# OFA-Sys/ONE-PEACE

Measured on NVIDIA H100. Metric: encoder_samples_per_sec, higher is better.
Workload: dtype bf16

## Files before the change

one_peace_b200/csrc/attention_wgmma.cu:

```cuda
#include "common.cuh"
#include "gemm.h"
#include "ops.h"

namespace opb {
namespace {

constexpr int kHd = 64;
constexpr int kThreads = 384;
constexpr int kStagerThreads = 96;
constexpr int kBoxRows = 32;
constexpr int kBoxBytes = kBoxRows * 128;
constexpr int kKeyChunks = kAttnShortMaxS / 32;

constexpr int kOffQ = 0;
constexpr int kOffK = kOffQ + 4 * 64 * 128;
constexpr int kOffV = kOffK + kAttnShortMaxS * 128;
constexpr int kOffLut = kOffV + kAttnShortMaxS * 128;
constexpr int kOffPad = kOffLut + kAttnShortMaxLut * 4;
constexpr int kBufBytes = (kOffPad + kAttnShortMaxS + 1023) / 1024 * 1024;
constexpr int kOffCodes = 2 * kBufBytes;
constexpr int kOffBars = kOffCodes + 2 * kAttnShortMaxS * 4;
constexpr int kSmemBytes = kOffBars + 64 + 1024;
static_assert(kSmemBytes <= 227 * 1024, "one CTA per SM");

enum BiasForm : int { kNoBias = 0, kDense = 1, kLut = 2, kLutSeg = 3 };

struct ShortArgs {
  const float* bias;
  long bias_bstride;
  int s_pad;
  LutBias lb;
  const uint8_t* key_pad;
  __nv_bfloat16* out;
  float* lse;
  float* ln_stats;
  int B, S, H;
};

OPB_DEVICE void wgmma_m64n32k16_ss(float (&d)[16], uint64_t desc_a, uint64_t desc_b, uint32_t scale_d) {
  asm volatile(
      "{\n\t"
      ".reg .pred p;\n\t"
      "setp.ne.b32 p, %18, 0;\n\t"
      "wgmma.mma_async.sync.aligned.m64n32k16.f32.bf16.bf16 "
      "{%0, %1, %2, %3, %4, %5, %6, %7, %8, %9, %10, %11, %12, %13, %14, %15}, %16, %17, p, 1, 1, 0, 0;\n\t"
      "}\n"
      : "+f"(d[0]), "+f"(d[1]), "+f"(d[2]), "+f"(d[3]), "+f"(d[4]), "+f"(d[5]), "+f"(d[6]), "+f"(d[7]),
        "+f"(d[8]), "+f"(d[9]), "+f"(d[10]), "+f"(d[11]), "+f"(d[12]), "+f"(d[13]), "+f"(d[14]), "+f"(d[15])
      : "l"(desc_a), "l"(desc_b), "r"(scale_d));
}

OPB_DEVICE void wgmma_m64n64k16_rs(float (&d)[32], const uint32_t (&a)[4], uint64_t desc_b, uint32_t scale_d) {
  asm volatile(
      "{\n\t"
      ".reg .pred p;\n\t"
      "setp.ne.b32 p, %37, 0;\n\t"
      "wgmma.mma_async.sync.aligned.m64n64k16.f32.bf16.bf16 "
      "{%0, %1, %2, %3, %4, %5, %6, %7, %8, %9, %10, %11, %12, %13, %14, %15, "
      "%16, %17, %18, %19, %20, %21, %22, %23, %24, %25, %26, %27, %28, %29, %30, %31}, "
      "{%32, %33, %34, %35}, %36, p, 1, 1, 1;\n\t"
      "}\n"
      : "+f"(d[0]), "+f"(d[1]), "+f"(d[2]), "+f"(d[3]), "+f"(d[4]), "+f"(d[5]), "+f"(d[6]), "+f"(d[7]),
        "+f"(d[8]), "+f"(d[9]), "+f"(d[10]), "+f"(d[11]), "+f"(d[12]), "+f"(d[13]), "+f"(d[14]), "+f"(d[15]),
        "+f"(d[16]), "+f"(d[17]), "+f"(d[18]), "+f"(d[19]), "+f"(d[20]), "+f"(d[21]), "+f"(d[22]), "+f"(d[23]),
        "+f"(d[24]), "+f"(d[25]), "+f"(d[26]), "+f"(d[27]), "+f"(d[28]), "+f"(d[29]), "+f"(d[30]), "+f"(d[31])
      : "r"(a[0]), "r"(a[1]), "r"(a[2]), "r"(a[3]), "l"(desc_b), "r"(scale_d));
}

template <int N>
OPB_DEVICE void fence_regs(float (&d)[N]) {
#pragma unroll
  for (int i = 0; i < N; ++i) asm volatile("" : "+f"(d[i])::"memory");
}

OPB_DEVICE float quad_max(float v) {
  v = fmaxf(v, __shfl_xor_sync(0xffffffffu, v, 1));
  return fmaxf(v, __shfl_xor_sync(0xffffffffu, v, 2));
}
OPB_DEVICE float quad_sum(float v) {
  v += __shfl_xor_sync(0xffffffffu, v, 1);
  return v + __shfl_xor_sync(0xffffffffu, v, 2);
}

OPB_DEVICE void load_bias_chunk(float2 (&dst)[4][2], const float* bias_lo, const float* bias_hi, int c, int t, int S) {
#pragma unroll
  for (int j = 0; j < 4; ++j) {
    const int key = (4 * c + j) * 8 + 2 * t;
    dst[j][0] = key < S ? *reinterpret_cast<const float2*>(bias_lo + key) : make_float2(0.f, 0.f);
    dst[j][1] = key < S ? *reinterpret_cast<const float2*>(bias_hi + key) : make_float2(0.f, 0.f);
  }
}

template <int kForm, int kChunks>
OPB_DEVICE void attend_tile(const ShortArgs& a, const uint8_t* buf, const int* code_row_s, const int* code_col_s, int b,
                            int h, int qt) {
  const int S = a.S, D = a.H * kHd;
  const int warp = (threadIdx.x >> 5) & 3, lane = threadIdx.x & 31;
  const int g = lane >> 2, t = lane & 3;
  const int row_lo = qt * 64 + warp * 16 + g, row_hi = row_lo + 8;
  const int rl = row_lo < S ? row_lo : 0, rh = row_hi < S ? row_hi : 0;
  const bool warp_live = qt * 64 + warp * 16 < S;

  const float* bias_lo = nullptr;
  const float* bias_hi = nullptr;
  float2 pre[2][4][2];
  if (kForm == kDense && warp_live) {
    bias_lo = a.bias + b * a.bias_bstride + (static_cast<long>(h) * S + rl) * a.s_pad;
    bias_hi = a.bias + b * a.bias_bstride + (static_cast<long>(h) * S + rh) * a.s_pad;
    load_bias_chunk(pre[0], bias_lo, bias_hi, 0, t, S);
    if (kChunks > 1) load_bias_chunk(pre[1], bias_lo, bias_hi, 1, t, S);
  }

  float s[kChunks][16];
  const uint32_t q_addr = smem_u32(buf + kOffQ) + qt * 8192;
  const uint32_t k_addr = smem_u32(buf + kOffK);
  wgmma_fence();
#pragma unroll
  for (int c = 0; c < kChunks; ++c) {
#pragma unroll
    for (int k = 0; k < 4; ++k)
      wgmma_m64n32k16_ss(s[c], wgmma_desc_sw128(q_addr + 32 * k, 8192), wgmma_desc_sw128(k_addr + c * 4096 + 32 * k, 8192),
                         k > 0 ? 1u : 0u);
  }
  wgmma_commit();
  wgmma_wait<0>();
#pragma unroll
  for (int c = 0; c < kChunks; ++c) fence_regs(s[c]);

  float mx_lo = -INFINITY, mx_hi = -INFINITY, sum_lo = 0.f, sum_hi = 0.f;
  uint32_t pf[4 * kChunks][2];
  if (warp_live) {
    const uint8_t* kp = a.key_pad != nullptr ? buf + kOffPad : nullptr;
    const float* lut_s = reinterpret_cast<const float*>(buf + kOffLut);
    const int crow_lo = kForm >= kLut ? code_row_s[rl] : 0;
    const int crow_hi = kForm >= kLut ? code_row_s[rh] : 0;
    const int seg = a.lb.seg_split;
    const bool first_lo = rl < seg, first_hi = rh < seg;
#pragma unroll
    for (int nt = 0; nt < 4 * kChunks; ++nt) {
      const int c = nt >> 2, e = (nt & 3) * 4;
      const int key = nt * 8 + 2 * t;
      float b00 = 0.f, b01 = 0.f, b10 = 0.f, b11 = 0.f;
      if (kForm == kDense) {
        if ((nt & 3) == 0) __syncwarp();
        const float2 x = pre[c & 1][nt & 3][0], y = pre[c & 1][nt & 3][1];
        b00 = x.x; b01 = x.y; b10 = y.x; b11 = y.y;
        if ((nt & 3) == 3 && c + 2 < kChunks) load_bias_chunk(pre[c & 1], bias_lo, bias_hi, c + 2, t, S);
      } else if (kForm == kLut) {
        const int2 cc = *reinterpret_cast<const int2*>(code_col_s + key);
        b00 = lut_s[crow_lo - cc.x]; b01 = lut_s[crow_lo - cc.y];
        b10 = lut_s[crow_hi - cc.x]; b11 = lut_s[crow_hi - cc.y];
      } else if (kForm == kLutSeg) {
        const int2 cc = *reinterpret_cast<const int2*>(code_col_s + key);
        const bool kf0 = key < seg, kf1 = key + 1 < seg;
        const bool s00 = first_lo == kf0, s01 = first_lo == kf1, s10 = first_hi == kf0, s11 = first_hi == kf1;
        b00 = lut_s[s00 ? crow_lo - cc.x : 0]; b01 = lut_s[s01 ? crow_lo - cc.y : 0];
        b10 = lut_s[s10 ? crow_hi - cc.x : 0]; b11 = lut_s[s11 ? crow_hi - cc.y : 0];
        b00 = s00 ? b00 : 0.f; b01 = s01 ? b01 : 0.f;
        b10 = s10 ? b10 : 0.f; b11 = s11 ? b11 : 0.f;
      }
      bool dead0 = key >= S, dead1 = key + 1 >= S;
      if (kp != nullptr) {
        const uint32_t pair = *reinterpret_cast<const uint16_t*>(kp + key);
        dead0 = dead0 || (pair & 0xffu) != 0;
        dead1 = dead1 || (pair >> 8) != 0;
      }
      s[c][e + 0] = dead0 ? -INFINITY : s[c][e + 0] + b00;
      s[c][e + 1] = dead1 ? -INFINITY : s[c][e + 1] + b01;
      s[c][e + 2] = dead0 ? -INFINITY : s[c][e + 2] + b10;
      s[c][e + 3] = dead1 ? -INFINITY : s[c][e + 3] + b11;
      mx_lo = fmaxf(mx_lo, fmaxf(s[c][e + 0], s[c][e + 1]));
      mx_hi = fmaxf(mx_hi, fmaxf(s[c][e + 2], s[c][e + 3]));
    }
    mx_lo = quad_max(mx_lo);
    mx_hi = quad_max(mx_hi);

    const float base_lo = (mx_lo == -INFINITY) ? 0.f : mx_lo;
    const float base_hi = (mx_hi == -INFINITY) ? 0.f : mx_hi;
#pragma unroll
    for (int nt = 0; nt < 4 * kChunks; ++nt) {
      const int c = nt >> 2, e = (nt & 3) * 4;
      const float p0 = __expf(s[c][e + 0] - base_lo), p1 = __expf(s[c][e + 1] - base_lo);
      const float p2 = __expf(s[c][e + 2] - base_hi), p3 = __expf(s[c][e + 3] - base_hi);
      sum_lo += p0 + p1;
      sum_hi += p2 + p3;
      pf[nt][0] = pack_bf16x2(p0, p1);
      pf[nt][1] = pack_bf16x2(p2, p3);
    }
  } else {
#pragma unroll
    for (int nt = 0; nt < 4 * kChunks; ++nt) pf[nt][0] = pf[nt][1] = 0u;
  }

  float o[32];
  const uint32_t v_addr = smem_u32(buf + kOffV);
#pragma unroll
  for (int nt = 0; nt < 4 * kChunks; ++nt) asm volatile("" : "+r"(pf[nt][0]), "+r"(pf[nt][1])::"memory");
  fence_regs(o);
  wgmma_fence();
#pragma unroll
  for (int kk = 0; kk < 2 * kChunks; ++kk) {
    const uint32_t af[4] = {pf[2 * kk][0], pf[2 * kk][1], pf[2 * kk + 1][0], pf[2 * kk + 1][1]};
    wgmma_m64n64k16_rs(o, af, wgmma_desc_sw128(v_addr + kk * 2048, 8192), kk > 0 ? 1u : 0u);
  }
  wgmma_commit();
  wgmma_wait<0>();
  fence_regs(o);

  const float l_lo = quad_sum(sum_lo), l_hi = quad_sum(sum_hi);
  const float inv_lo = l_lo > 0.f ? 1.f / l_lo : 0.f;
  const float inv_hi = l_hi > 0.f ? 1.f / l_hi : 0.f;
  const long rows_total = static_cast<long>(a.B) * S;
  if (a.ln_stats != nullptr) {
    float s_lo = 0.f, q_lo = 0.f, s_hi = 0.f, q_hi = 0.f;
#pragma unroll
    for (int nd = 0; nd < 8; ++nd) {
      const float a0 = o[4 * nd] * inv_lo, a1 = o[4 * nd + 1] * inv_lo;
      const float a2 = o[4 * nd + 2] * inv_hi, a3 = o[4 * nd + 3] * inv_hi;
      s_lo += a0 + a1; q_lo += a0 * a0 + a1 * a1;
      s_hi += a2 + a3; q_hi += a2 * a2 + a3 * a3;
    }
    s_lo = quad_sum(s_lo); q_lo = quad_sum(q_lo);
    s_hi = quad_sum(s_hi); q_hi = quad_sum(q_hi);
    if (t == 0 && row_lo < S)
      *reinterpret_cast<float2*>(a.ln_stats + (h * rows_total + static_cast<long>(b) * S + row_lo) * 2) = make_float2(s_lo, q_lo);
    if (t == 0 && row_hi < S)
      *reinterpret_cast<float2*>(a.ln_stats + (h * rows_total + static_cast<long>(b) * S + row_hi) * 2) = make_float2(s_hi, q_hi);
  }
  if (row_lo < S) {
    __nv_bfloat16* op = a.out + (static_cast<long>(b) * S + row_lo) * D + h * kHd + 2 * t;
#pragma unroll
    for (int nd = 0; nd < 8; ++nd)
      *reinterpret_cast<uint32_t*>(op + nd * 8) = pack_bf16x2(o[4 * nd] * inv_lo, o[4 * nd + 1] * inv_lo);
    if (a.lse != nullptr && t == 0) a.lse[(static_cast<long>(b) * a.H + h) * S + row_lo] = mx_lo + __logf(l_lo);
  }
  if (row_hi < S) {
    __nv_bfloat16* op = a.out + (static_cast<long>(b) * S + row_hi) * D + h * kHd + 2 * t;
#pragma unroll
    for (int nd = 0; nd < 8; ++nd)
      *reinterpret_cast<uint32_t*>(op + nd * 8) = pack_bf16x2(o[4 * nd + 2] * inv_hi, o[4 * nd + 3] * inv_hi);
    if (a.lse != nullptr && t == 0) a.lse[(static_cast<long>(b) * a.H + h) * S + row_hi] = mx_hi + __logf(l_hi);
  }
}

template <int kForm, int kChunks>
__global__ void __launch_bounds__(kThreads, 1)
attention_short_kernel(const __grid_constant__ CUtensorMap tm_qkv, const ShortArgs a) {
  extern __shared__ uint8_t smem_raw[];
  uint8_t* smem = smem_raw + ((1024u - (smem_u32(smem_raw) & 1023u)) & 1023u);
  int* code_row_s = reinterpret_cast<int*>(smem + kOffCodes);
  int* code_col_s = code_row_s + kAttnShortMaxS;
  uint64_t* full = reinterpret_cast<uint64_t*>(smem + kOffBars);
  uint64_t* empty = full + 2;

  const int S = a.S, H = a.H, D = H * kHd;
  const int units = a.B * H;
  const int n_qt = (S + 63) / 64;
  const int wg = threadIdx.x >> 7;

  if (threadIdx.x == 0) {
    tma_prefetch_desc(&tm_qkv);
    for (int i = 0; i < 2; ++i) {
      mbar_init(&full[i], 1 + kStagerThreads);
      mbar_init(&empty[i], 8);
    }
    fence_barrier_init();
  }
  if (kForm >= kLut) {
    for (int i = threadIdx.x; i < kAttnShortMaxS; i += kThreads) {
      if (i < S) code_row_s[i] = a.lb.code_row[i];
      code_col_s[i] = a.lb.code_col[i < S ? i : S - 1];
    }
  }
  __syncthreads();

  if (wg == 0) {
    asm volatile("setmaxnreg.dec.sync.aligned.u32 40;");
    if (threadIdx.x == 0) {
      uint32_t j = 0;
      for (int unit = blockIdx.x; unit < units; unit += gridDim.x, ++j) {
        const int b = unit / H, h = unit - b * H;
        uint8_t* buf = smem + (j & 1) * kBufBytes;
        mbar_wait_quiet(&empty[j & 1], ((j >> 1) & 1) ^ 1);
        mbar_arrive_expect_tx(&full[j & 1], 3 * kChunks * kBoxBytes);
        for (int i = 0; i < kChunks; ++i) {
          tma_load_3d(&tm_qkv, &full[j & 1], buf + kOffQ + i * kBoxBytes, h * kHd, i * kBoxRows, b);
          tma_load_3d(&tm_qkv, &full[j & 1], buf + kOffK + i * kBoxBytes, D + h * kHd, i * kBoxRows, b);
          tma_load_3d(&tm_qkv, &full[j & 1], buf + kOffV + i * kBoxBytes, 2 * D + h * kHd, i * kBoxRows, b);
        }
      }
    } else if (threadIdx.x >= 32) {
      const int t = threadIdx.x - 32;
      uint32_t j = 0;
      for (int unit = blockIdx.x; unit < units; unit += gridDim.x, ++j) {
        const int b = unit / H, h = unit - b * H;
        uint8_t* buf = smem + (j & 1) * kBufBytes;
        mbar_wait_quiet(&empty[j & 1], ((j >> 1) & 1) ^ 1);
        if (kForm >= kLut) {
          const float* src = a.lb.lut + static_cast<long>(h) * a.lb.lut_len;
          float* dst = reinterpret_cast<float*>(buf + kOffLut);
          for (int i = t; i < a.lb.lut_len; i += kStagerThreads) dst[i] = src[i];
        }
        if (a.key_pad != nullptr) {
          const uint8_t* src = a.key_pad + static_cast<long>(b) * S;
          for (int i = t; i < S; i += kStagerThreads) buf[kOffPad + i] = src[i];
        }
        mbar_arrive(&full[j & 1]);
      }
    }
  } else {
    asm volatile("setmaxnreg.inc.sync.aligned.u32 232;");
    const int cw = wg - 1;
    uint32_t j = 0;
    for (int unit = blockIdx.x; unit < units; unit += gridDim.x, ++j) {
      const int b = unit / H, h = unit - b * H;
      const uint8_t* buf = smem + (j & 1) * kBufBytes;
      mbar_wait_quiet(&full[j & 1], (j >> 1) & 1);
      for (int qt = cw; qt < n_qt; qt += 2) attend_tile<kForm, kChunks>(a, buf, code_row_s, code_col_s, b, h, qt);
      __syncwarp();
      if ((threadIdx.x & 31) == 0) mbar_arrive(&empty[j & 1]);
    }
  }
}

template <int kForm, int kChunks>
int launch_short(const CUtensorMap& tm, const ShortArgs& a, cudaStream_t stream) {
  auto kern = attention_short_kernel<kForm, kChunks>;
  static bool attr_set = false;
  if (!attr_set) {
    if (cudaFuncSetAttribute(kern, cudaFuncAttributeMaxDynamicSharedMemorySize, kSmemBytes) != cudaSuccess)
      return OPB_ERR_CUDA;
    attr_set = true;
  }
  const int units = a.B * a.H;
  const int grid = units < sm_count() ? units : sm_count();
  kern<<<grid, kThreads, kSmemBytes, stream>>>(tm, a);
  return cudaGetLastError() == cudaSuccess ? OPB_OK : OPB_ERR_CUDA;
}

template <int kForm>
int launch_form(const CUtensorMap& tm, const ShortArgs& a, cudaStream_t stream) {
  static_assert(kKeyChunks == 7, "one case per chunk count");
  switch ((a.S + 31) / 32) {
    case 1: return launch_short<kForm, 1>(tm, a, stream);
    case 2: return launch_short<kForm, 2>(tm, a, stream);
    case 3: return launch_short<kForm, 3>(tm, a, stream);
    case 4: return launch_short<kForm, 4>(tm, a, stream);
    case 5: return launch_short<kForm, 5>(tm, a, stream);
    case 6: return launch_short<kForm, 6>(tm, a, stream);
    case 7: return launch_short<kForm, 7>(tm, a, stream);
    default: return OPB_ERR_INVALID;
  }
}

}

int attention_fwd_short(const void* qkv, const float* bias, const uint8_t* key_pad, void* out, float* lse, float* ln_stats,
                        int B, int S, int H, int s_pad, long bias_bstride, const LutBias& lb, cudaStream_t stream) {
  if (B <= 0 || S <= 0 || H <= 0 || S > kAttnShortMaxS || lb.lut_len > kAttnShortMaxLut) return OPB_ERR_INVALID;
  const uint64_t D = static_cast<uint64_t>(H) * kHd;
  CUtensorMap tm;
  const int rc = make_tmap_bf16_batched(&tm, qkv, 3 * D, S, 3 * D, B, S * 3 * D, kBoxRows);
  if (rc != OPB_OK) return rc;
  ShortArgs a;
  a.bias = bias; a.bias_bstride = bias_bstride; a.s_pad = s_pad; a.lb = lb;
  a.key_pad = key_pad;
  a.out = reinterpret_cast<__nv_bfloat16*>(out); a.lse = lse; a.ln_stats = ln_stats;
  a.B = B; a.S = S; a.H = H;
  if (bias != nullptr) return launch_form<kDense>(tm, a, stream);
  if (lb.lut != nullptr) return lb.seg_split > 0 ? launch_form<kLutSeg>(tm, a, stream) : launch_form<kLut>(tm, a, stream);
  return launch_form<kNoBias>(tm, a, stream);
}

}
```

one_peace_b200/csrc/common.cuh:

```cuda
#pragma once
#include <cuda.h>
#include <cuda_bf16.h>
#include <cuda_runtime.h>
#include <stdint.h>
#include <stdio.h>
#include <stdlib.h>

#define OPB_DEVICE __device__ __forceinline__

#define OPB_OK 0
#define OPB_ERR_INVALID 1
#define OPB_ERR_CUDA 2
#define OPB_ERR_UNSUPPORTED 3

namespace opb {

OPB_DEVICE uint32_t smem_u32(const void* p) {
  return static_cast<uint32_t>(__cvta_generic_to_shared(p));
}
OPB_DEVICE uint32_t lane_id() { return threadIdx.x & 31; }

OPB_DEVICE bool elect_one() {
  uint32_t pred = 0;
  asm volatile(
      "{\n\t"
      ".reg .pred P;\n\t"
      "elect.sync _|P, 0xffffffff;\n\t"
      "selp.b32 %0, 1, 0, P;\n\t"
      "}\n"
      : "=r"(pred));
  return pred != 0;
}

OPB_DEVICE uint64_t globaltimer_ns() {
  uint64_t t;
  asm volatile("mov.u64 %0, %%globaltimer;" : "=l"(t));
  return t;
}

OPB_DEVICE void mbar_init(uint64_t* bar, uint32_t count) {
  asm volatile("mbarrier.init.shared::cta.b64 [%0], %1;" ::"r"(smem_u32(bar)), "r"(count) : "memory");
}
OPB_DEVICE void fence_barrier_init() { asm volatile("fence.mbarrier_init.release.cluster;" ::: "memory"); }
OPB_DEVICE void fence_proxy_async() { asm volatile("fence.proxy.async.shared::cta;" ::: "memory"); }

OPB_DEVICE void mbar_arrive_expect_tx(uint64_t* bar, uint32_t bytes) {
  asm volatile("mbarrier.arrive.expect_tx.shared::cta.b64 _, [%0], %1;" ::"r"(smem_u32(bar)), "r"(bytes)
               : "memory");
}
OPB_DEVICE void mbar_arrive(uint64_t* bar) {
  asm volatile("mbarrier.arrive.shared::cta.b64 _, [%0];" ::"r"(smem_u32(bar)) : "memory");
}
OPB_DEVICE void mbar_arrive_count(uint64_t* bar, uint32_t count) {
  asm volatile("mbarrier.arrive.shared::cta.b64 _, [%0], %1;" ::"r"(smem_u32(bar)), "r"(count) : "memory");
}
OPB_DEVICE bool mbar_try_wait(uint64_t* bar, uint32_t parity) {
  uint32_t ok;
  asm volatile(
      "{\n\t"
      ".reg .pred P;\n\t"
      "mbarrier.try_wait.parity.shared::cta.b64 P, [%1], %2;\n\t"
      "selp.b32 %0, 1, 0, P;\n\t"
      "}\n"
      : "=r"(ok)
      : "r"(smem_u32(bar)), "r"(parity)
      : "memory");
  return ok != 0;
}

#ifndef OPB_WATCHDOG_NS
#define OPB_WATCHDOG_NS 4000000000ull
#endif
OPB_DEVICE void mbar_wait(uint64_t* bar, uint32_t parity) {
  if (mbar_try_wait(bar, parity)) return;
  uint64_t t0 = globaltimer_ns();
  uint32_t spins = 0;
  while (!mbar_try_wait(bar, parity)) {
    if ((++spins & 0x3ff) == 0) {
      if (globaltimer_ns() - t0 > OPB_WATCHDOG_NS) {
        printf("[opb] mbarrier watchdog: block %d thread %d bar@%u parity %u\n", (int)blockIdx.x,
               (int)threadIdx.x, smem_u32(bar), parity);
        __trap();
      }
    }
  }
}

OPB_DEVICE void mbar_wait_quiet(uint64_t* bar, uint32_t parity) {
  if (mbar_try_wait(bar, parity)) return;
  const uint64_t t0 = globaltimer_ns();
  while (!mbar_try_wait(bar, parity)) {
    if (globaltimer_ns() - t0 > OPB_WATCHDOG_NS) __trap();
  }
}

OPB_DEVICE uint64_t wgmma_desc_sw128(uint32_t smem_addr, uint32_t lbo) {
  uint64_t d = 0;
  d |= static_cast<uint64_t>((smem_addr & 0x3FFFFu) >> 4);
  d |= static_cast<uint64_t>((lbo >> 4) & 0x3FFFu) << 16;
  d |= static_cast<uint64_t>(1024 >> 4) << 32;
  d |= static_cast<uint64_t>(1) << 62;
  return d;
}

OPB_DEVICE void wgmma_fence() { asm volatile("wgmma.fence.sync.aligned;" ::: "memory"); }
OPB_DEVICE void wgmma_commit() { asm volatile("wgmma.commit_group.sync.aligned;" ::: "memory"); }
template <int N>
OPB_DEVICE void wgmma_wait() { asm volatile("wgmma.wait_group.sync.aligned %0;" ::"n"(N) : "memory"); }

static inline int sm_count() {
  static int n = 0;
  if (n == 0) {
    int dev = 0;
    cudaGetDevice(&dev);
    cudaDeviceGetAttribute(&n, cudaDevAttrMultiProcessorCount, dev);
  }
  return n;
}

OPB_DEVICE void tma_prefetch_desc(const CUtensorMap* m) {
  asm volatile("prefetch.tensormap [%0];" ::"l"(reinterpret_cast<uint64_t>(m)) : "memory");
}

OPB_DEVICE void tma_load_2d(const CUtensorMap* m, uint64_t* bar, void* dst, int32_t c0, int32_t c1) {
  asm volatile(
      "cp.async.bulk.tensor.2d.shared::cluster.global.mbarrier::complete_tx::bytes [%0], [%1, {%3, %4}], [%2];"
      :
      : "r"(smem_u32(dst)), "l"(reinterpret_cast<uint64_t>(m)), "r"(smem_u32(bar)), "r"(c0), "r"(c1)
      : "memory");
}
OPB_DEVICE void tma_load_3d(const CUtensorMap* m, uint64_t* bar, void* dst, int32_t c0, int32_t c1, int32_t c2) {
  asm volatile(
      "cp.async.bulk.tensor.3d.shared::cluster.global.mbarrier::complete_tx::bytes [%0], [%1, {%3, %4, %5}], [%2];"
      :
      : "r"(smem_u32(dst)), "l"(reinterpret_cast<uint64_t>(m)), "r"(smem_u32(bar)), "r"(c0), "r"(c1), "r"(c2)
      : "memory");
}
OPB_DEVICE void bulk_load_1d(void* dst, const void* src, uint32_t bytes, uint64_t* bar) {
  asm volatile("cp.async.bulk.shared::cluster.global.mbarrier::complete_tx::bytes [%0], [%1], %2, [%3];" ::"r"(smem_u32(dst)),
               "l"(reinterpret_cast<uint64_t>(src)), "r"(bytes), "r"(smem_u32(bar))
               : "memory");
}

OPB_DEVICE void tma_store_2d(const CUtensorMap* m, const void* src, int32_t c0, int32_t c1) {
  asm volatile("cp.async.bulk.tensor.2d.global.shared::cta.bulk_group [%0, {%2, %3}], [%1];" ::"l"(
                   reinterpret_cast<uint64_t>(m)),
               "r"(smem_u32(src)), "r"(c0), "r"(c1)
               : "memory");
}
OPB_DEVICE void bulk_commit() { asm volatile("cp.async.bulk.commit_group;" ::: "memory"); }
template <int N>
OPB_DEVICE void bulk_wait_read() { asm volatile("cp.async.bulk.wait_group.read %0;" ::"n"(N) : "memory"); }
template <int N>
OPB_DEVICE void bulk_wait_all() { asm volatile("cp.async.bulk.wait_group %0;" ::"n"(N) : "memory"); }

OPB_DEVICE uint32_t sw64_off(int row, int chunk) { return row * 64 + ((chunk ^ ((row >> 1) & 3)) << 4); }
OPB_DEVICE uint32_t sw128_off(int row, int chunk) { return row * 128 + ((chunk ^ (row & 7)) << 4); }

OPB_DEVICE float fast_erf(float x) {
  const float ax = fabsf(x);
  float t;
  asm("rcp.approx.ftz.f32 %0, %1;" : "=f"(t) : "f"(fmaf(0.3275911f, ax, 1.0f)));
  float p = fmaf(1.061405429f, t, -1.453152027f);
  p = fmaf(p, t, 1.421413741f);
  p = fmaf(p, t, -0.284496736f);
  p = fmaf(p, t, 0.254829592f);
  p *= t;
  float e;
  asm("ex2.approx.ftz.f32 %0, %1;" : "=f"(e) : "f"(-1.4426950408889634f * ax * ax));
  const float r = fmaf(-p, e, 1.0f);
  return copysignf(r, x);
}
OPB_DEVICE float gelu_erf(float x) { return 0.5f * x * (1.0f + fast_erf(x * 0.70710678118654752440f)); }

OPB_DEVICE float4 lds128(const uint8_t* p) { return *reinterpret_cast<const float4*>(p); }
OPB_DEVICE void sts128(uint8_t* p, float4 v) { *reinterpret_cast<float4*>(p) = v; }
OPB_DEVICE void sts128u(uint8_t* p, uint4 v) { *reinterpret_cast<uint4*>(p) = v; }

OPB_DEVICE uint32_t pack_bf16x2(float lo, float hi) {
  __nv_bfloat162 v = __floats2bfloat162_rn(lo, hi);
  return *reinterpret_cast<uint32_t*>(&v);
}
OPB_DEVICE float2 unpack_bf16x2(uint32_t u) {
  __nv_bfloat162 v = *reinterpret_cast<__nv_bfloat162*>(&u);
  return __bfloat1622float2(v);
}

OPB_DEVICE float warp_sum(float v) {
#pragma unroll
  for (int o = 16; o > 0; o >>= 1) v += __shfl_xor_sync(0xffffffffu, v, o);
  return v;
}
OPB_DEVICE float warp_max(float v) {
#pragma unroll
  for (int o = 16; o > 0; o >>= 1) v = fmaxf(v, __shfl_xor_sync(0xffffffffu, v, o));
  return v;
}

}
```

Before: 830.0.

## Store attention output via stmatrix and TMA, specialize key-pad masking

The attention output epilogue now writes each 64-row tile into the consumed Q buffer in shared memory with stmatrix using a 128B swizzle, then issues one TMA 3D store per warpgroup in place of scattered 4-byte global stores. The bias/mask loop is also split into compile-time variants with and without key padding, and the out-of-range key check is limited to the last chunk. LUT addressing is simplified, and q-tile assignment alternates between consumer warpgroups across units. The change adds a named barrier and a bulk wait before releasing the buffer, and it relies on the TMA box clipping rows past S.

New measurement: 833.9 (median of 6 runs). About the same (+0.5%).

```diff
diff --git a/one_peace_b200/csrc/attention_wgmma.cu b/one_peace_b200/csrc/attention_wgmma.cu
--- a/one_peace_b200/csrc/attention_wgmma.cu
+++ b/one_peace_b200/csrc/attention_wgmma.cu
@@ -1,3 +1,5 @@
+#include <type_traits>
+
 #include "common.cuh"
 #include "gemm.h"
 #include "ops.h"
@@ -92,9 +94,9 @@
 }
 
 template <int kForm, int kChunks>
-OPB_DEVICE void attend_tile(const ShortArgs& a, const uint8_t* buf, const int* code_row_s, const int* code_col_s, int b,
-                            int h, int qt) {
-  const int S = a.S, D = a.H * kHd;
+OPB_DEVICE void attend_tile(const CUtensorMap& tm_out, const ShortArgs& a, const uint8_t* buf, const int* code_row_s,
+                            const int* code_col_s, int b, int h, int qt) {
+  const int S = a.S;
   const int warp = (threadIdx.x >> 5) & 3, lane = threadIdx.x & 31;
   const int g = lane >> 2, t = lane & 3;
   const int row_lo = qt * 64 + warp * 16 + g, row_hi = row_lo + 8;
@@ -136,42 +138,50 @@
     const int crow_hi = kForm >= kLut ? code_row_s[rh] : 0;
     const int seg = a.lb.seg_split;
     const bool first_lo = rl < seg, first_hi = rh < seg;
-#pragma unroll
-    for (int nt = 0; nt < 4 * kChunks; ++nt) {
-      const int c = nt >> 2, e = (nt & 3) * 4;
-      const int key = nt * 8 + 2 * t;
-      float b00 = 0.f, b01 = 0.f, b10 = 0.f, b11 = 0.f;
-      if (kForm == kDense) {
-        if ((nt & 3) == 0) __syncwarp();
-        const float2 x = pre[c & 1][nt & 3][0], y = pre[c & 1][nt & 3][1];
-        b00 = x.x; b01 = x.y; b10 = y.x; b11 = y.y;
-        if ((nt & 3) == 3 && c + 2 < kChunks) load_bias_chunk(pre[c & 1], bias_lo, bias_hi, c + 2, t, S);
-      } else if (kForm == kLut) {
-        const int2 cc = *reinterpret_cast<const int2*>(code_col_s + key);
-        b00 = lut_s[crow_lo - cc.x]; b01 = lut_s[crow_lo - cc.y];
-        b10 = lut_s[crow_hi - cc.x]; b11 = lut_s[crow_hi - cc.y];
-      } else if (kForm == kLutSeg) {
-        const int2 cc = *reinterpret_cast<const int2*>(code_col_s + key);
-        const bool kf0 = key < seg, kf1 = key + 1 < seg;
-        const bool s00 = first_lo == kf0, s01 = first_lo == kf1, s10 = first_hi == kf0, s11 = first_hi == kf1;
-        b00 = lut_s[s00 ? crow_lo - cc.x : 0]; b01 = lut_s[s01 ? crow_lo - cc.y : 0];
-        b10 = lut_s[s10 ? crow_hi - cc.x : 0]; b11 = lut_s[s11 ? crow_hi - cc.y : 0];
-        b00 = s00 ? b00 : 0.f; b01 = s01 ? b01 : 0.f;
-        b10 = s10 ? b10 : 0.f; b11 = s11 ? b11 : 0.f;
+    const float* lut_lo = lut_s + crow_lo;
+    const float* lut_hi = lut_s + crow_hi;
+    auto bias_mask_max = [&](auto has_pad) {
+      const bool pad = has_pad;
+#pragma unroll
+      for (int nt = 0; nt < 4 * kChunks; ++nt) {
+        const int c = nt >> 2, e = (nt & 3) * 4;
+        const int key = nt * 8 + 2 * t;
+        float b00 = 0.f, b01 = 0.f, b10 = 0.f, b11 = 0.f;
+        if (kForm == kDense) {
+          if ((nt & 3) == 0) __syncwarp();
+          const float2 x = pre[c & 1][nt & 3][0], y = pre[c & 1][nt & 3][1];
+          b00 = x.x; b01 = x.y; b10 = y.x; b11 = y.y;
+          if ((nt & 3) == 3 && c + 2 < kChunks) load_bias_chunk(pre[c & 1], bias_lo, bias_hi, c + 2, t, S);
+        } else if (kForm == kLut) {
+          const int2 cc = *reinterpret_cast<const int2*>(code_col_s + key);
+          b00 = lut_lo[-cc.x]; b01 = lut_lo[-cc.y];
+          b10 = lut_hi[-cc.x]; b11 = lut_hi[-cc.y];
+        } else if (kForm == kLutSeg) {
+          const int2 cc = *reinterpret_cast<const int2*>(code_col_s + key);
+          const bool kf0 = key < seg, kf1 = key + 1 < seg;
+          const bool s00 = first_lo == kf0, s01 = first_lo == kf1, s10 = first_hi == kf0, s11 = first_hi == kf1;
+          b00 = *(s00 ? lut_lo - cc.x : lut_s); b01 = *(s01 ? lut_lo - cc.y : lut_s);
+          b10 = *(s10 ? lut_hi - cc.x : lut_s); b11 = *(s11 ? lut_hi - cc.y : lut_s);
+          b00 = s00 ? b00 : 0.f; b01 = s01 ? b01 : 0.f;
+          b10 = s10 ? b10 : 0.f; b11 = s11 ? b11 : 0.f;
+        }
+        bool dead0 = c == kChunks - 1 && key >= S, dead1 = c == kChunks - 1 && key + 1 >= S;
+        if (pad) {
+          const uint32_t pair = *reinterpret_cast<const uint16_t*>(kp + key);
+          dead0 = dead0 || (pair & 0xffu) != 0;
+          dead1 = dead1 || (pair >> 8) != 0;
+        }
+        s[c][e + 0] = dead0 ? -INFINITY : s[c][e + 0] + b00;
+        s[c][e + 1] = dead1 ? -INFINITY : s[c][e + 1] + b01;
+        s[c][e + 2] = dead0 ? -INFINITY : s[c][e + 2] + b10;
+        s[c][e + 3] = dead1 ? -INFINITY : s[c][e + 3] + b11;
+        mx_lo = fmaxf(mx_lo, fmaxf(s[c][e + 0], s[c][e + 1]));
+        mx_hi = fmaxf(mx_hi, fmaxf(s[c][e + 2], s[c][e + 3]));
       }
-      bool dead0 = key >= S, dead1 = key + 1 >= S;
-      if (kp != nullptr) {
-        const uint32_t pair = *reinterpret_cast<const uint16_t*>(kp + key);
-        dead0 = dead0 || (pair & 0xffu) != 0;
-        dead1 = dead1 || (pair >> 8) != 0;
-      }
-      s[c][e + 0] = dead0 ? -INFINITY : s[c][e + 0] + b00;
-      s[c][e + 1] = dead1 ? -INFINITY : s[c][e + 1] + b01;
-      s[c][e + 2] = dead0 ? -INFINITY : s[c][e + 2] + b10;
-      s[c][e + 3] = dead1 ? -INFINITY : s[c][e + 3] + b11;
-      mx_lo = fmaxf(mx_lo, fmaxf(s[c][e + 0], s[c][e + 1]));
-      mx_hi = fmaxf(mx_hi, fmaxf(s[c][e + 2], s[c][e + 3]));
-    }
+    };
+    if constexpr (kForm == kDense) bias_mask_max(kp != nullptr);
+    else if (kp != nullptr) bias_mask_max(std::true_type{});
+    else bias_mask_max(std::false_type{});
     mx_lo = quad_max(mx_lo);
     mx_hi = quad_max(mx_hi);
 
@@ -227,25 +237,39 @@
     if (t == 0 && row_hi < S)
       *reinterpret_cast<float2*>(a.ln_stats + (h * rows_total + static_cast<long>(b) * S + row_hi) * 2) = make_float2(s_hi, q_hi);
   }
-  if (row_lo < S) {
-    __nv_bfloat16* op = a.out + (static_cast<long>(b) * S + row_lo) * D + h * kHd + 2 * t;
-#pragma unroll
-    for (int nd = 0; nd < 8; ++nd)
-      *reinterpret_cast<uint32_t*>(op + nd * 8) = pack_bf16x2(o[4 * nd] * inv_lo, o[4 * nd + 1] * inv_lo);
-    if (a.lse != nullptr && t == 0) a.lse[(static_cast<long>(b) * a.H + h) * S + row_lo] = mx_lo + __logf(l_lo);
-  }
-  if (row_hi < S) {
-    __nv_bfloat16* op = a.out + (static_cast<long>(b) * S + row_hi) * D + h * kHd + 2 * t;
-#pragma unroll
-    for (int nd = 0; nd < 8; ++nd)
-      *reinterpret_cast<uint32_t*>(op + nd * 8) = pack_bf16x2(o[4 * nd + 2] * inv_hi, o[4 * nd + 3] * inv_hi);
-    if (a.lse != nullptr && t == 0) a.lse[(static_cast<long>(b) * a.H + h) * S + row_hi] = mx_hi + __logf(l_hi);
+  if (a.lse != nullptr && t == 0) {
+    if (row_lo < S) a.lse[(static_cast<long>(b) * a.H + h) * S + row_lo] = mx_lo + __logf(l_lo);
+    if (row_hi < S) a.lse[(static_cast<long>(b) * a.H + h) * S + row_hi] = mx_hi + __logf(l_hi);
+  }
+
+  uint8_t* stage = const_cast<uint8_t*>(buf) + kOffQ + qt * 8192;
+#pragma unroll
+  for (int half = 0; half < 2; ++half) {
+    const float inv = half ? inv_hi : inv_lo;
+    const int row = warp * 16 + 8 * half + (lane & 7);
+#pragma unroll
+    for (int q = 0; q < 2; ++q) {
+      uint32_t v[4];
+#pragma unroll
+      for (int i = 0; i < 4; ++i) v[i] = pack_bf16x2(o[4 * (4 * q + i) + 2 * half] * inv, o[4 * (4 * q + i) + 2 * half + 1] * inv);
+      const uint32_t addr = smem_u32(stage) + sw128_off(row, 4 * q + (lane >> 3));
+      asm volatile("stmatrix.sync.aligned.m8n8.x4.shared.b16 [%0], {%1, %2, %3, %4};" ::"r"(addr), "r"(v[0]), "r"(v[1]),
+                   "r"(v[2]), "r"(v[3]));
+    }
+  }
+  fence_proxy_async();
+  if (threadIdx.x >> 7 == 1) asm volatile("bar.sync 1, 128;" ::: "memory");
+  else asm volatile("bar.sync 2, 128;" ::: "memory");
+  if ((threadIdx.x & 127) == 0) {
+    tma_store_3d(&tm_out, stage, h * kHd, qt * 64, b);
+    bulk_commit();
   }
 }
 
 template <int kForm, int kChunks>
 __global__ void __launch_bounds__(kThreads, 1)
-attention_short_kernel(const __grid_constant__ CUtensorMap tm_qkv, const ShortArgs a) {
+attention_short_kernel(const __grid_constant__ CUtensorMap tm_qkv, const __grid_constant__ CUtensorMap tm_out,
+                       const ShortArgs a) {
   extern __shared__ uint8_t smem_raw[];
   uint8_t* smem = smem_raw + ((1024u - (smem_u32(smem_raw) & 1023u)) & 1023u);
   int* code_row_s = reinterpret_cast<int*>(smem + kOffCodes);
@@ -260,6 +284,7 @@
 
   if (threadIdx.x == 0) {
     tma_prefetch_desc(&tm_qkv);
+    tma_prefetch_desc(&tm_out);
     for (int i = 0; i < 2; ++i) {
       mbar_init(&full[i], 1 + kStagerThreads);
       mbar_init(&empty[i], 8);
@@ -316,7 +341,9 @@
       const int b = unit / H, h = unit - b * H;
       const uint8_t* buf = smem + (j & 1) * kBufBytes;
       mbar_wait_quiet(&full[j & 1], (j >> 1) & 1);
-      for (int qt = cw; qt < n_qt; qt += 2) attend_tile<kForm, kChunks>(a, buf, code_row_s, code_col_s, b, h, qt);
+      for (int qt = (cw + j) & 1; qt < n_qt; qt += 2)
+        attend_tile<kForm, kChunks>(tm_out, a, buf, code_row_s, code_col_s, b, h, qt);
+      if ((threadIdx.x & 127) == 0) bulk_wait_read<0>();
       __syncwarp();
       if ((threadIdx.x & 31) == 0) mbar_arrive(&empty[j & 1]);
     }
@@ -324,7 +351,7 @@
 }
 
 template <int kForm, int kChunks>
-int launch_short(const CUtensorMap& tm, const ShortArgs& a, cudaStream_t stream) {
+int launch_short(const CUtensorMap& tm, const CUtensorMap& tm_out, const ShortArgs& a, cudaStream_t stream) {
   auto kern = attention_short_kernel<kForm, kChunks>;
   static bool attr_set = false;
   if (!attr_set) {
@@ -334,21 +361,21 @@
   }
   const int units = a.B * a.H;
   const int grid = units < sm_count() ? units : sm_count();
-  kern<<<grid, kThreads, kSmemBytes, stream>>>(tm, a);
+  kern<<<grid, kThreads, kSmemBytes, stream>>>(tm, tm_out, a);
   return cudaGetLastError() == cudaSuccess ? OPB_OK : OPB_ERR_CUDA;
 }
 
 template <int kForm>
-int launch_form(const CUtensorMap& tm, const ShortArgs& a, cudaStream_t stream) {
+int launch_form(const CUtensorMap& tm, const CUtensorMap& tm_out, const ShortArgs& a, cudaStream_t stream) {
   static_assert(kKeyChunks == 7, "one case per chunk count");
   switch ((a.S + 31) / 32) {
-    case 1: return launch_short<kForm, 1>(tm, a, stream);
-    case 2: return launch_short<kForm, 2>(tm, a, stream);
-    case 3: return launch_short<kForm, 3>(tm, a, stream);
-    case 4: return launch_short<kForm, 4>(tm, a, stream);
-    case 5: return launch_short<kForm, 5>(tm, a, stream);
-    case 6: return launch_short<kForm, 6>(tm, a, stream);
-    case 7: return launch_short<kForm, 7>(tm, a, stream);
+    case 1: return launch_short<kForm, 1>(tm, tm_out, a, stream);
+    case 2: return launch_short<kForm, 2>(tm, tm_out, a, stream);
+    case 3: return launch_short<kForm, 3>(tm, tm_out, a, stream);
+    case 4: return launch_short<kForm, 4>(tm, tm_out, a, stream);
+    case 5: return launch_short<kForm, 5>(tm, tm_out, a, stream);
+    case 6: return launch_short<kForm, 6>(tm, tm_out, a, stream);
+    case 7: return launch_short<kForm, 7>(tm, tm_out, a, stream);
     default: return OPB_ERR_INVALID;
   }
 }
@@ -360,16 +387,20 @@
   if (B <= 0 || S <= 0 || H <= 0 || S > kAttnShortMaxS || lb.lut_len > kAttnShortMaxLut) return OPB_ERR_INVALID;
   const uint64_t D = static_cast<uint64_t>(H) * kHd;
   CUtensorMap tm;
-  const int rc = make_tmap_bf16_batched(&tm, qkv, 3 * D, S, 3 * D, B, S * 3 * D, kBoxRows);
+  int rc = make_tmap_bf16_batched(&tm, qkv, 3 * D, S, 3 * D, B, S * 3 * D, kBoxRows);
+  if (rc != OPB_OK) return rc;
+  CUtensorMap tm_out;
+  rc = make_tmap_bf16_batched(&tm_out, out, D, S, D, B, S * D, 64);
   if (rc != OPB_OK) return rc;
   ShortArgs a;
   a.bias = bias; a.bias_bstride = bias_bstride; a.s_pad = s_pad; a.lb = lb;
   a.key_pad = key_pad;
   a.out = reinterpret_cast<__nv_bfloat16*>(out); a.lse = lse; a.ln_stats = ln_stats;
   a.B = B; a.S = S; a.H = H;
-  if (bias != nullptr) return launch_form<kDense>(tm, a, stream);
-  if (lb.lut != nullptr) return lb.seg_split > 0 ? launch_form<kLutSeg>(tm, a, stream) : launch_form<kLut>(tm, a, stream);
-  return launch_form<kNoBias>(tm, a, stream);
-}
-
-}
+  if (bias != nullptr) return launch_form<kDense>(tm, tm_out, a, stream);
+  if (lb.lut != nullptr)
+    return lb.seg_split > 0 ? launch_form<kLutSeg>(tm, tm_out, a, stream) : launch_form<kLut>(tm, tm_out, a, stream);
+  return launch_form<kNoBias>(tm, tm_out, a, stream);
+}
+
+}
diff --git a/one_peace_b200/csrc/common.cuh b/one_peace_b200/csrc/common.cuh
--- a/one_peace_b200/csrc/common.cuh
+++ b/one_peace_b200/csrc/common.cuh
@@ -148,6 +148,12 @@
                "r"(smem_u32(src)), "r"(c0), "r"(c1)
                : "memory");
 }
+OPB_DEVICE void tma_store_3d(const CUtensorMap* m, const void* src, int32_t c0, int32_t c1, int32_t c2) {
+  asm volatile("cp.async.bulk.tensor.3d.global.shared::cta.bulk_group [%0, {%2, %3, %4}], [%1];" ::"l"(
+                   reinterpret_cast<uint64_t>(m)),
+               "r"(smem_u32(src)), "r"(c0), "r"(c1), "r"(c2)
+               : "memory");
+}
 OPB_DEVICE void bulk_commit() { asm volatile("cp.async.bulk.commit_group;" ::: "memory"); }
 template <int N>
 OPB_DEVICE void bulk_wait_read() { asm volatile("cp.async.bulk.wait_group.read %0;" ::"n"(N) : "memory"); }
```
